# leftfield-geospatial/homonim

Measured on AMD Instinct MI355X. Metric: Mpixels*bands/s fit+apply (5x5 gain-offset, float32), higher is better.
Workload: dtype f32 in/out, f64 window sums; 1 GPU; synthetic float32 4-band 16384x16384 src/ref resident in HBM per GPU, Model.gain-offset, kernel 5x5, r2_inpaint_thresh 0.25, fused fit+apply (BASELINE.json configs[2]); bands=4, height=16384, width=16384, nodata_variant=0, parallelism=1 rank(s) x 1 GPU, one raster per rank, no collective

## Files before the change

### homonim_amd/csrc/hk_norm.hip

```cpp
#include "hk_kernels.h"

#include <type_traits>

namespace hk {

constexpr int NORM_THREADS = 256;
constexpr int L1_BITS = 11, L2_BITS = 11, L3_BITS = 10;
constexpr int L1_BINS = 1 << L1_BITS, L2_BINS = 1 << L2_BITS, L3_BINS = 1 << L3_BITS;
constexpr int SAMPLE_N = 4096;
#ifndef HK_NORM_ABLATE
#define HK_NORM_ABLATE 0
#endif
constexpr int PASS_WAVES = 2048;
constexpr int FB_BLOCKS = 512;
constexpr int MID_BLOCKS = 256;

struct Sel {
    unsigned prefix;
    unsigned long long rank;
};

struct NormWS {
    float lo[2], hi[2];
    double shift[2];
    unsigned sample_m;
    unsigned long long pn[PASS_WAVES], pbelow[2][PASS_WAVES];
    double p1[2][PASS_WAVES], p2[2][PASS_WAVES];
    unsigned mid_count[2];
    unsigned long long n;
    double mean[2], var[2], frac;
    unsigned long long k[2];
    int fallback, done;
    Sel sel[2][2];
    unsigned kbase[2];
    int ksh[2];
    float val[2][2];
    unsigned hist1[2][2][L1_BINS], hist2[2][2][L2_BINS], hist3[2][2][L3_BINS];
};

static_assert(sizeof(NormWS) == NORM_WS_BYTES, "the workspace's per-band piece (hk_layout.h)");

size_t norm_workspace_bytes(int n_bands, int height, int width) { return norm_layout(n_bands, height, width).total; }
static float* mid_buffers(void* workspace, const NormLayout& l) { return reinterpret_cast<float*>(static_cast<char*>(workspace) + l.mid); }

__device__ __forceinline__ unsigned f2key(float f) {
    const unsigned u = __float_as_uint(f);
    return (u & 0x80000000u) ? ~u : (u | 0x80000000u);
}
__device__ __forceinline__ float key2f(unsigned k) {
    const unsigned u = (k & 0x80000000u) ? (k & 0x7fffffffu) : ~k;
    return __uint_as_float(u);
}
__device__ __forceinline__ bool nvalid(float v, int mode, float nodata) {
    return mode == 0 ? true : (mode == 1 ? !(v != v) : !(v == nodata));
}

struct PlaneRef {
    const float* sp;
    const float* rp;
    long long stride;
    int height, width;
};
__device__ __forceinline__ PlaneRef plane_of(const NormArgs& a, int p) {
    PlaneRef r;
    if (a.planes != nullptr) {
        const __attribute__((address_space(1))) NormPlane* const e = (const __attribute__((address_space(1))) NormPlane*)a.planes + p;
        r.sp = e->src, r.rp = e->ref, r.stride = e->stride, r.height = e->height, r.width = e->width;
    } else {
        r.sp = a.src + (long long)p * a.band_stride, r.rp = a.ref + (long long)p * a.band_stride;
        r.stride = a.stride, r.height = a.height, r.width = a.width;
    }
    return r;
}

__device__ __forceinline__ float plane_at(const float* plane, long long i) {
    return *((__attribute__((address_space(1))) const float*)plane + i);
}

__device__ __forceinline__ double wave_sum(double v) {
#pragma unroll
    for (int d = WAVE / 2; d > 0; d >>= 1) v += __shfl_xor(v, d);
    return v;
}
__device__ __forceinline__ unsigned long long wave_sum(unsigned long long v) {
#pragma unroll
    for (int d = WAVE / 2; d > 0; d >>= 1) v += __shfl_xor(v, d);
    return v;
}

template <int NBINS, typename T = unsigned>
__device__ __forceinline__ bool select_bin(const T* __restrict__ h, unsigned long long rank, unsigned* bin_out,
                                           unsigned long long* rank_out) {
    const int lane = threadIdx.x & (WAVE - 1);
    constexpr int PER = NBINS / WAVE;
    unsigned v[PER];
    unsigned long long local = 0;
#pragma unroll
    for (int i = 0; i < PER; ++i) v[i] = h[lane * PER + i];
#pragma unroll
    for (int i = 0; i < PER; ++i) local += v[i];
    unsigned long long incl = local;
#pragma unroll
    for (int d = 1; d < WAVE; d <<= 1) {
        const unsigned long long u = __shfl_up(incl, d, WAVE);
        if (lane >= d) incl += u;
    }
    const unsigned long long hit = __ballot(incl > rank);
    const int owner = hit ? __ffsll(hit) - 1 : WAVE - 1;
    if (lane != owner) return false;
    unsigned long long cum = incl - local;
    int b = 0;
    bool found = false;
#pragma unroll
    for (int i = 0; i < PER - 1; ++i) {
        if (!found) {
            if (cum + v[i] > rank) found = true;
            else cum += v[i], b = i + 1;
        }
    }
    *bin_out = (unsigned)(lane * PER + b);
    *rank_out = rank - cum;
    return true;
}

constexpr int SAMPLE_THREADS = 256;
__global__ void __launch_bounds__(SAMPLE_THREADS) norm_sample_kernel(const NormArgs a, NormWS* __restrict__ ws_all) {
    static_assert(L1_BINS == L2_BINS && L3_BINS <= L1_BINS, "the sample select shares one histogram shape");
    static_assert(SAMPLE_N < 65536, "16-bit histogram counters");
    __shared__ float samp[SAMPLE_N];
    __shared__ unsigned hist[2][L1_BINS / 2];
    __shared__ unsigned cnt, spfx[2], srank[2];
    __shared__ int need[2];
    __shared__ double red[SAMPLE_THREADS / WAVE];
    const int band = blockIdx.x, t = threadIdx.x;
    NormWS& ws = ws_all[band];
    const PlaneRef pl = plane_of(a, band);
    const float* __restrict__ sp = pl.sp;
    const float* __restrict__ rp = pl.rp;
    const long long total = (long long)pl.height * pl.width;
    const long long step = total / SAMPLE_N > 0 ? total / SAMPLE_N : 1;
    for (int q = 0; q < 2; ++q) {
        if (t == 0) cnt = 0;
        for (int i = t; i < SAMPLE_N; i += SAMPLE_THREADS) samp[i] = __int_as_float(0x7f800000);
        __syncthreads();
        double sum = 0.0;
        for (int j = t; j < SAMPLE_N; j += SAMPLE_THREADS) {
            unsigned long long hsh = ((unsigned long long)j + 0x9e3779b97f4a7c15ull) * 0xbf58476d1ce4e5b9ull;
            hsh = (hsh ^ (hsh >> 29)) * 0x94d049bb133111ebull;
            hsh ^= hsh >> 32;
            const long long p = (long long)j * step + (long long)(hsh % (unsigned long long)step);
            if (p < total) {
                const int y = (int)(p / pl.width), x = (int)(p % pl.width);
                const float s = plane_at(sp, (long long)y * pl.stride + x), r = plane_at(rp, (long long)y * pl.stride + x);
                if (nvalid(s, a.src_nd_mode, a.src_nodata) && nvalid(r, a.ref_nd_mode, a.ref_nodata)) {
                    const float v = q ? r : s;
                    samp[atomicAdd(&cnt, 1u)] = v;
                    sum += (double)v;
                }
            }
        }
        __syncthreads();
        const unsigned m = cnt;
        {
            const double wsum = wave_sum(sum);
            if ((t & (WAVE - 1)) == 0) red[t / WAVE] = wsum;
        }
        if (t == 0) {
            const double c = 0.01 * (double)m, sd = sqrt(c > 0.0 ? c : 0.0);
            const long long ia = (long long)floor(c - 4.0 * sd) - 2, ib = (long long)ceil(c + 4.0 * sd) + 3;
            need[0] = !(m == 0 || ia <= 0), need[1] = !(m == 0 || ib >= (long long)m - 1);
            srank[0] = need[0] ? (unsigned)ia : 0u, srank[1] = need[1] ? (unsigned)ib : 0u;
            spfx[0] = spfx[1] = 0u;
        }
        __syncthreads();
        for (int level = 0; level < 3; ++level) {
            for (int i = t; i < L1_BINS; i += SAMPLE_THREADS) (&hist[0][0])[i] = 0;
            __syncthreads();
            for (int i = t; i < SAMPLE_N; i += SAMPLE_THREADS) {
                const unsigned key = f2key(samp[i]);
#pragma unroll
                for (int k = 0; k < 2; ++k) {
                    unsigned bin;
                    bool in;
                    if (level == 0) bin = key >> (32 - L1_BITS), in = true;
                    else if (level == 1) bin = (key >> L3_BITS) & (L2_BINS - 1), in = (key >> (32 - L1_BITS)) == spfx[k];
                    else bin = key & (L3_BINS - 1), in = (key >> L3_BITS) == spfx[k];
                    if (in) atomicAdd(&hist[k][bin >> 1], 1u << (16 * (bin & 1u)));
                }
            }
            __syncthreads();
            if (t < 2 * WAVE) {
                const int k = t / WAVE;
                const unsigned short* h16 = reinterpret_cast<const unsigned short*>(hist[k]);
                unsigned bin;
                unsigned long long rk;
                bool mine;
                if (level == 2) mine = select_bin<L3_BINS, unsigned short>(h16, srank[k], &bin, &rk);
                else mine = select_bin<L1_BINS, unsigned short>(h16, srank[k], &bin, &rk);
                if (mine) {
                    const int bits = level == 0 ? 0 : (level == 1 ? L2_BITS : L3_BITS);
                    spfx[k] = level == 0 ? bin : ((spfx[k] << bits) | bin);
                    srank[k] = (unsigned)rk;
                }
            }
            __syncthreads();
        }
        if (t == 0) {
            double s_all = 0.0;
            for (int i = 0; i < SAMPLE_THREADS / WAVE; ++i) s_all += red[i];
            const double mean = m ? s_all / (double)m : 0.0;
            ws.shift[q] = (mean == mean && fabs(mean) < 1e300) ? mean : 0.0;
            ws.sample_m = m;
            const float lo = key2f(spfx[0]), hi = key2f(spfx[1]);
            ws.lo[q] = need[0] ? (lo == 0.0f ? -0.0f : lo) : __int_as_float(0xff800000);
            ws.hi[q] = need[1] ? (hi == 0.0f ? 0.0f : hi) : __int_as_float(0x7f800000);
        }
        __syncthreads();
    }
}

constexpr size_t NORM_STREAM_LDS_PAD = 0;

__host__ __device__ static inline int pass_waves(int height, int width) {
    const long long chunks = (long long)height * (((width + PX - 1) / PX + WAVE - 1) / WAVE);
    long long w = chunks / 16;
    w = w < 64 ? 64 : (w > PASS_WAVES ? PASS_WAVES : w);
    return (int)w;
}

constexpr int QCAP = 16;

template <bool DENSE>
__global__ void __launch_bounds__(WAVE) norm_stream_kernel(const NormArgs a, NormWS* __restrict__ ws_all,
                                                            float* __restrict__ mid_all, size_t mid_cap) {
    __shared__ float stage[2][QCAP][WAVE];
    const int band = blockIdx.y, wave = blockIdx.x, lane = threadIdx.x;
    NormWS& ws = ws_all[band];
    const PlaneRef pl = plane_of(a, band);
    const int G = pass_waves(pl.height, pl.width);
    if (wave >= G) return;
    const float* __restrict__ sp = pl.sp;
    const float* __restrict__ rp = pl.rp;
    float* mid[2] = {mid_all + ((size_t)band * 2 + 0) * mid_cap, mid_all + ((size_t)band * 2 + 1) * mid_cap};
    const float lo[2] = {ws.lo[0], ws.lo[1]}, hi[2] = {ws.hi[0], ws.hi[1]};
    const double shift[2] = {ws.shift[0], ws.shift[1]};

    unsigned n = 0, le_hi[2] = {0, 0}, n_in[2] = {0, 0};
    double m1[2] = {0.0, 0.0}, m2[2] = {0.0, 0.0};
    unsigned cnt[2] = {0, 0};

    auto flush = [&](int q) {
        unsigned incl = cnt[q];
#pragma unroll
        for (int d = 1; d < WAVE; d <<= 1) {
            const unsigned v = __shfl_up(incl, d, WAVE);
            if (lane >= d) incl += v;
        }
        const unsigned total = __shfl(incl, WAVE - 1);
        unsigned base = 0;
        if (lane == 0) base = atomicAdd(&ws.mid_count[q], total);
        base = __shfl(base, 0);
        const size_t off = (size_t)base + (incl - cnt[q]);
        for (unsigned j = 0; j < cnt[q]; ++j)
            if (off + j < mid_cap) mid[q][off + j] = stage[q][j][lane];
        n_in[q] += cnt[q];
        cnt[q] = 0;
    };

    const int wq = (pl.width + PX - 1) / PX, cpr = (wq + WAVE - 1) / WAVE;
    const long long total = (long long)pl.height * cpr;
    const int dy = G / cpr, dc = G % cpr;
    int py = wave / cpr, pc = wave % cpr;
    long long pit = wave;
    auto fetch = [&](float4& s4, float4& r4, int& x) {
        const bool live = pit < total;
        const long long o = live ? (long long)py * pl.stride + (long long)pc * (WAVE * PX) : 0ll;
        const bool ok = live && pc * WAVE + lane < wq;
        const int lo4 = ok ? lane * PX : 0;
        typedef float f4v __attribute__((ext_vector_type(4)));
        typedef __attribute__((address_space(1))) const f4v gf4v;
        const f4v sv = __builtin_nontemporal_load((gf4v*)(sp + o + lo4));
        const f4v rv = __builtin_nontemporal_load((gf4v*)(rp + o + lo4));
        s4 = make_float4(sv.x, sv.y, sv.z, sv.w), r4 = make_float4(rv.x, rv.y, rv.z, rv.w);
        x = ok ? (pc * WAVE + lane) * PX : pl.width;
        pit += G, py += dy, pc += dc;
        if (pc >= cpr) pc -= cpr, ++py;
    };
    const float cmp_s = a.src_nd_mode == 2 ? a.src_nodata : __int_as_float(0x7fc00000);
    const float cmp_r = a.ref_nd_mode == 2 ? a.ref_nodata : __int_as_float(0x7fc00000);
    const bool nan_s = a.src_nd_mode == 1, nan_r = a.ref_nd_mode == 1;
    auto process = [&](const float4& s4, const float4& r4, int x, auto full) {
        constexpr bool FULL = decltype(full)::value;
        if (__any((cnt[0] > cnt[1] ? cnt[0] : cnt[1]) > (unsigned)(QCAP - PX))) {
            if (__any(cnt[0] > (unsigned)(QCAP - PX))) flush(0);
            if (__any(cnt[1] > (unsigned)(QCAP - PX))) flush(1);
        }
        const float s[PX] = {s4.x, s4.y, s4.z, s4.w}, r[PX] = {r4.x, r4.y, r4.z, r4.w};
        const int npx = pl.width - x;
#pragma unroll
        for (int i = 0; i < PX; ++i) {
            bool m = FULL || i < npx;
            if constexpr (!DENSE)
                m = m && !(s[i] == cmp_s) && !(r[i] == cmp_r) && (s[i] == s[i] || !nan_s) && (r[i] == r[i] || !nan_r);
            const float v[2] = {s[i], r[i]};
            if (m) {
                ++n;
#pragma unroll
                for (int q = 0; q < 2; ++q) {
                    if constexpr ((HK_NORM_ABLATE & 1) != 0) { m1[q] += (double)(v[q] == 1.2345f); continue; }
                    const double d = (double)v[q] - shift[q];
                    m1[q] += d;
                    m2[q] = __fma_rn(d, d, m2[q]);
                }
            }
#pragma unroll
            for (int q = 0; q < 2; ++q) {
                if constexpr ((HK_NORM_ABLATE & 2) != 0) { le_hi[q] += (m && v[q] <= hi[q]) ? 1u : 0u; continue; }
                const bool le = m && v[q] <= hi[q], in = le && !(v[q] < lo[q]);
                stage[q][cnt[q]][lane] = v[q];
                le_hi[q] += le ? 1u : 0u;
                cnt[q] += in ? 1u : 0u;
            }
        }
    };
    const bool quads = (pl.width % PX) == 0;
    auto process_any = [&](const float4& s4, const float4& r4, int x) {
        if (quads && __shfl(x, WAVE - 1) < pl.width) process(s4, r4, x, std::true_type{});
        else process(s4, r4, x, std::false_type{});
    };

    constexpr int NS = 3;
    float4 sQ[NS], rQ[NS];
    int xQ[NS];
#pragma unroll
    for (int k = 0; k < NS; ++k) fetch(sQ[k], rQ[k], xQ[k]);
    for (long long it = wave; it < total;) {
        bool more = true;
#pragma unroll
        for (int k = 0; k < NS; ++k) {
            if (more) {
                process_any(sQ[k], rQ[k], xQ[k]);
                fetch(sQ[k], rQ[k], xQ[k]);
                more = (it += G) < total;
            }
        }
    }
    flush(0);
    flush(1);
    const unsigned long long nw = wave_sum((unsigned long long)n);
    unsigned long long bw[2];
    for (int q = 0; q < 2; ++q) {
        m1[q] = wave_sum(m1[q]);
        m2[q] = wave_sum(m2[q]);
        bw[q] = wave_sum((unsigned long long)(le_hi[q] - n_in[q]));
    }
    if (lane == 0) {
        ws.pn[wave] = nw;
        for (int q = 0; q < 2; ++q) ws.p1[q][wave] = m1[q], ws.p2[q][wave] = m2[q], ws.pbelow[q][wave] = bw[q];
    }
}

constexpr int STATS_THREADS = 256;
__global__ void __launch_bounds__(STATS_THREADS) norm_stats_kernel(NormWS* __restrict__ ws_all, double* __restrict__ norm_out,
                                                                    size_t mid_cap) {
    static_assert(PASS_WAVES % STATS_THREADS == 0, "every thread sums the same number of partials");
    __shared__ unsigned long long sn[STATS_THREADS / WAVE], sb[2][STATS_THREADS / WAVE];
    __shared__ double s1[2][STATS_THREADS / WAVE], s2[2][STATS_THREADS / WAVE];
    NormWS& ws = ws_all[blockIdx.x];
    unsigned long long n = 0, below[2] = {0, 0};
    double m1[2] = {0.0, 0.0}, m2[2] = {0.0, 0.0};
#pragma unroll
    for (int j = 0; j < PASS_WAVES / STATS_THREADS; ++j) {
        const int i = threadIdx.x + j * STATS_THREADS;
        n += ws.pn[i];
#pragma unroll
        for (int q = 0; q < 2; ++q) m1[q] += ws.p1[q][i], m2[q] += ws.p2[q][i], below[q] += ws.pbelow[q][i];
    }
    n = wave_sum(n);
    for (int q = 0; q < 2; ++q) m1[q] = wave_sum(m1[q]), m2[q] = wave_sum(m2[q]), below[q] = wave_sum(below[q]);
    const int w = threadIdx.x / WAVE;
    if ((threadIdx.x & (WAVE - 1)) == 0) {
        sn[w] = n;
        for (int q = 0; q < 2; ++q) s1[q][w] = m1[q], s2[q][w] = m2[q], sb[q][w] = below[q];
    }
    __syncthreads();
    if (threadIdx.x != 0) return;
    n = 0;
    for (int q = 0; q < 2; ++q) m1[q] = m2[q] = 0.0, below[q] = 0;
    for (int i = 0; i < STATS_THREADS / WAVE; ++i) {
        n += sn[i];
        for (int q = 0; q < 2; ++q) m1[q] += s1[q][i], m2[q] += s2[q][i], below[q] += sb[q][i];
    }
    ws.n = n;
    if (n == 0) {
        norm_out[2 * blockIdx.x] = 0.0;
        norm_out[2 * blockIdx.x + 1] = 0.0;
        ws.done = 1;
        return;
    }
    for (int q = 0; q < 2; ++q) {
        const double d = m1[q] / (double)n;
        ws.mean[q] = ws.shift[q] + d;
        const double v = m2[q] / (double)n - d * d;
        ws.var[q] = v > 0.0 ? v : 0.0;
    }
    const double vi = 0.01 * (double)(n - 1);
    const unsigned long long k0 = (unsigned long long)floor(vi);
    ws.frac = vi - (double)k0;
    ws.k[0] = k0;
    ws.k[1] = k0 + 1 < n ? k0 + 1 : n - 1;
    int fb = 0;
    for (int q = 0; q < 2; ++q) {
        const unsigned long long nm = ws.mid_count[q];
        if (nm > mid_cap || ws.k[0] < below[q] || ws.k[1] >= below[q] + nm) fb = 1;
        ws.sel[q][0].rank = ws.k[0] - below[q];
        ws.sel[q][1].rank = ws.k[1] - below[q];
        ws.sel[q][0].prefix = ws.sel[q][1].prefix = 0;
        const unsigned kb = f2key(ws.lo[q]), range = f2key(ws.hi[q]) - kb;
        ws.kbase[q] = kb;
        ws.ksh[q] = range ? __clz((int)range) : 0;
    }
    if (fb)
        for (int q = 0; q < 2; ++q) {
            ws.sel[q][0].rank = ws.k[0], ws.sel[q][1].rank = ws.k[1];
            ws.kbase[q] = 0, ws.ksh[q] = 0;
        }
    ws.fallback = fb;
}

__device__ __forceinline__ void hist_add(unsigned* hist, int level, unsigned key, const unsigned (&pfx)[2]) {
    if (level == 0) {
        atomicAdd(&hist[key >> (32 - L1_BITS)], 1u);
        return;
    }
#pragma unroll
    for (int k = 0; k < 2; ++k) {
        if (level == 1) {
            if ((key >> (32 - L1_BITS)) == pfx[k]) atomicAdd(&hist[k * L2_BINS + ((key >> L3_BITS) & (L2_BINS - 1))], 1u);
        } else {
            if ((key >> L3_BITS) == pfx[k]) atomicAdd(&hist[k * L3_BINS + (key & (L3_BINS - 1))], 1u);
        }
    }
}

template <int LEVEL>
__global__ void __launch_bounds__(NORM_THREADS) norm_mid_hist_kernel(const NormArgs a, NormWS* __restrict__ ws_all,
                                                                       const float* __restrict__ mid_all, size_t mid_cap) {
    constexpr int NB = LEVEL == 0 ? L1_BINS : (LEVEL == 1 ? L2_BINS : L3_BINS);
    __shared__ unsigned hist[2 * NB];
    const int band = blockIdx.y >> 1, q = blockIdx.y & 1;
    NormWS& ws = ws_all[band];
    if (ws.done) return;
    for (int i = threadIdx.x; i < 2 * NB; i += NORM_THREADS) hist[i] = 0;
    __syncthreads();
    if (ws.fallback) {
        const PlaneRef pl = plane_of(a, band);
        const unsigned pfx[2] = {ws.sel[q][0].prefix, ws.sel[q][1].prefix};
        const unsigned kb = ws.kbase[q];
        const int ksh = ws.ksh[q];
        for (int y = blockIdx.x; y < pl.height; y += gridDim.x) {
            const long long row = (long long)y * pl.stride;
            for (int x = threadIdx.x; x < pl.width; x += NORM_THREADS) {
                const float s = plane_at(pl.sp, row + x), r = plane_at(pl.rp, row + x);
                if (nvalid(s, a.src_nd_mode, a.src_nodata) && nvalid(r, a.ref_nd_mode, a.ref_nodata))
                    hist_add(hist, LEVEL, (f2key(q ? r : s) - kb) << ksh, pfx);
            }
        }
        __syncthreads();
        unsigned* gh = LEVEL == 0 ? &ws.hist1[q][0][0] : (LEVEL == 1 ? &ws.hist2[q][0][0] : &ws.hist3[q][0][0]);
        for (int i = threadIdx.x; i < 2 * NB; i += NORM_THREADS)
            if (hist[i]) atomicAdd(gh + i, hist[i]);
        return;
    }
    const float* __restrict__ buf = mid_all + ((size_t)band * 2 + q) * mid_cap;
    const unsigned cnt = ws.mid_count[q];
    const unsigned pfx[2] = {ws.sel[q][0].prefix, ws.sel[q][1].prefix};
    const unsigned kb = ws.kbase[q];
    const int ksh = ws.ksh[q];
    auto rel = [&](float v) { return (f2key(v) - kb) << ksh; };
    const float4* __restrict__ buf4 = reinterpret_cast<const float4*>(buf);
    const unsigned cnt4 = cnt >> 2;
    for (unsigned i = blockIdx.x * NORM_THREADS + threadIdx.x; i < cnt4; i += gridDim.x * NORM_THREADS) {
        const float4 v = buf4[i];
        hist_add(hist, LEVEL, rel(v.x), pfx), hist_add(hist, LEVEL, rel(v.y), pfx);
        hist_add(hist, LEVEL, rel(v.z), pfx), hist_add(hist, LEVEL, rel(v.w), pfx);
    }
    if (blockIdx.x == 0 && threadIdx.x < (cnt & 3u)) hist_add(hist, LEVEL, rel(buf[(cnt & ~3u) + threadIdx.x]), pfx);
    __syncthreads();
    unsigned* gh = LEVEL == 0 ? &ws.hist1[q][0][0] : (LEVEL == 1 ? &ws.hist2[q][0][0] : &ws.hist3[q][0][0]);
    for (int i = threadIdx.x; i < 2 * NB; i += NORM_THREADS)
        if (hist[i]) atomicAdd(gh + i, hist[i]);
}

template <int LEVEL>
__global__ void __launch_bounds__(NORM_THREADS) norm_full_hist_kernel(const NormArgs a, NormWS* __restrict__ ws_all) {
    constexpr int NB = LEVEL == 0 ? L1_BINS : (LEVEL == 1 ? L2_BINS : L3_BINS);
    __shared__ unsigned hist[2 * NB];
    const int band = blockIdx.y, q = blockIdx.z;
    NormWS& ws = ws_all[band];
    if (ws.done || !ws.fallback) return;
    for (int i = threadIdx.x; i < 2 * NB; i += NORM_THREADS) hist[i] = 0;
    __syncthreads();
    const PlaneRef pl = plane_of(a, band);
    const float* __restrict__ sp = pl.sp;
    const float* __restrict__ rp = pl.rp;
    const unsigned pfx[2] = {ws.sel[q][0].prefix, ws.sel[q][1].prefix};
    const unsigned kb = ws.kbase[q];
    const int ksh = ws.ksh[q];
    for (int y = blockIdx.x; y < pl.height; y += gridDim.x) {
        const long long row = (long long)y * pl.stride;
        for (int x = threadIdx.x; x < pl.width; x += NORM_THREADS) {
            const float s = plane_at(sp, row + x), r = plane_at(rp, row + x);
            if (nvalid(s, a.src_nd_mode, a.src_nodata) && nvalid(r, a.ref_nd_mode, a.ref_nodata))
                hist_add(hist, LEVEL, (f2key(q ? r : s) - kb) << ksh, pfx);
        }
    }
    __syncthreads();
    unsigned* gh = LEVEL == 0 ? &ws.hist1[q][0][0] : (LEVEL == 1 ? &ws.hist2[q][0][0] : &ws.hist3[q][0][0]);
    for (int i = threadIdx.x; i < 2 * NB; i += NORM_THREADS)
        if (hist[i]) atomicAdd(gh + i, hist[i]);
}

template <int LEVEL>
__global__ void __launch_bounds__(NORM_THREADS) norm_select_kernel(NormWS* __restrict__ ws_all, double* __restrict__ norm_out) {
    static_assert(NORM_THREADS == 4 * WAVE, "one wave per (raster, rank)");
    NormWS& ws = ws_all[blockIdx.x];
    if (ws.done) return;
    {
        const int q = threadIdx.x >> 7, k = (threadIdx.x >> 6) & 1;
        const unsigned* h = LEVEL == 0 ? ws.hist1[q][0] : (LEVEL == 1 ? ws.hist2[q][k] : ws.hist3[q][k]);
        constexpr int NB = LEVEL == 0 ? L1_BINS : (LEVEL == 1 ? L2_BINS : L3_BINS);
        unsigned bin;
        unsigned long long rk;
        if (select_bin<NB>(h, ws.sel[q][k].rank, &bin, &rk)) {
            const int bits = LEVEL == 0 ? 0 : (LEVEL == 1 ? L2_BITS : L3_BITS);
            ws.sel[q][k].prefix = (LEVEL == 0) ? bin : ((ws.sel[q][k].prefix << bits) | bin);
            ws.sel[q][k].rank = rk;
            if (LEVEL == 2) ws.val[q][k] = key2f((ws.sel[q][k].prefix >> ws.ksh[q]) + ws.kbase[q]);
        }
    }
    __syncthreads();
    if (LEVEL == 2 && threadIdx.x == 0) {
        const double n0 = sqrt(ws.var[1]) / sqrt(ws.var[0]);
        double pct[2];
        for (int q = 0; q < 2; ++q) {
            const double lo = (double)ws.val[q][0], hi = (double)ws.val[q][1], t = ws.frac;
            const double d = hi - lo;
            pct[q] = t >= 0.5 ? hi - d * (1.0 - t) : lo + d * t;
        }
        norm_out[2 * blockIdx.x] = n0;
        norm_out[2 * blockIdx.x + 1] = pct[1] - pct[0] * n0;
    }
}

constexpr int SPLIT_XCHG = 4 * L1_BINS;

size_t norm_split_exchange_doubles(int n_bands) { return (size_t)n_bands * SPLIT_XCHG; }

__global__ void split_put_shift_kernel(NormWS* __restrict__ ws_all, double* __restrict__ xchg) {
    NormWS& ws = ws_all[blockIdx.x];
    double* x = xchg + (size_t)blockIdx.x * SPLIT_XCHG;
    for (int i = threadIdx.x; i < SPLIT_XCHG; i += blockDim.x) x[i] = i < 2 ? ws.shift[i] : (i == 2 && ws.sample_m ? 1.0 : 0.0);
}
__global__ void split_get_shift_kernel(NormWS* __restrict__ ws_all, const double* __restrict__ xchg) {
    if (threadIdx.x != 0) return;
    NormWS& ws = ws_all[blockIdx.x];
    const double* x = xchg + (size_t)blockIdx.x * SPLIT_XCHG;
    for (int q = 0; q < 2; ++q) {
        ws.shift[q] = x[2] > 0.0 ? x[q] / x[2] : 0.0;
        ws.lo[q] = ws.hi[q] = __int_as_float(0xff800000);
    }
}
__global__ void split_put_moments_kernel(NormWS* __restrict__ ws_all, double* __restrict__ xchg) {
    NormWS& ws = ws_all[blockIdx.x];
    unsigned long long n = 0;
    double m1[2] = {0.0, 0.0}, m2[2] = {0.0, 0.0};
    for (int i = threadIdx.x; i < PASS_WAVES; i += WAVE) {
        n += ws.pn[i];
        for (int q = 0; q < 2; ++q) m1[q] += ws.p1[q][i], m2[q] += ws.p2[q][i];
    }
    n = wave_sum(n);
    for (int q = 0; q < 2; ++q) m1[q] = wave_sum(m1[q]), m2[q] = wave_sum(m2[q]);
    if (threadIdx.x != 0) return;
    double* x = xchg + (size_t)blockIdx.x * SPLIT_XCHG;
    x[0] = (double)n, x[1] = m1[0], x[2] = m2[0], x[3] = m1[1], x[4] = m2[1];
}
__global__ void split_get_moments_kernel(NormWS* __restrict__ ws_all, const double* __restrict__ xchg,
                                         double* __restrict__ norm_out) {
    if (threadIdx.x != 0) return;
    NormWS& ws = ws_all[blockIdx.x];
    const double* x = xchg + (size_t)blockIdx.x * SPLIT_XCHG;
    const unsigned long long n = (unsigned long long)x[0];
    ws.n = n;
    ws.mid_count[0] = ws.mid_count[1] = 0;
    if (n == 0) {
        norm_out[2 * blockIdx.x] = 0.0, norm_out[2 * blockIdx.x + 1] = 0.0;
        ws.done = 1;
        return;
    }
    if (n >= (1ull << 32)) {
        const double qn = __longlong_as_double(0x7ff8000000000000ll);
        norm_out[2 * blockIdx.x] = qn, norm_out[2 * blockIdx.x + 1] = qn;
        ws.done = 1;
        return;
    }
    for (int q = 0; q < 2; ++q) {
        const double d = x[1 + 2 * q] / (double)n;
        ws.mean[q] = ws.shift[q] + d;
        const double v = x[2 + 2 * q] / (double)n - d * d;
        ws.var[q] = v > 0.0 ? v : 0.0;
    }
    const double vi = 0.01 * (double)(n - 1);
    const unsigned long long k0 = (unsigned long long)floor(vi);
    ws.frac = vi - (double)k0;
    ws.k[0] = k0, ws.k[1] = k0 + 1 < n ? k0 + 1 : n - 1;
    for (int q = 0; q < 2; ++q)
        for (int k = 0; k < 2; ++k) ws.sel[q][k].rank = ws.k[k], ws.sel[q][k].prefix = 0;
    ws.fallback = 1;
}
template <int LEVEL>
__global__ void split_hist_kernel(NormWS* __restrict__ ws_all, double* __restrict__ xchg, int put) {
    constexpr int NB = LEVEL == 0 ? L1_BINS : (LEVEL == 1 ? L2_BINS : L3_BINS);
    NormWS& ws = ws_all[blockIdx.x];
    unsigned* h = LEVEL == 0 ? &ws.hist1[0][0][0] : (LEVEL == 1 ? &ws.hist2[0][0][0] : &ws.hist3[0][0][0]);
    double* x = xchg + (size_t)blockIdx.x * SPLIT_XCHG;
    for (int i = threadIdx.x; i < SPLIT_XCHG; i += blockDim.x) {
        if (put) x[i] = i < 4 * NB ? (double)h[i] : 0.0;
        else if (i < 4 * NB) h[i] = (unsigned)x[i];
    }
}

hipError_t launch_block_norm_split(const NormArgs& a, void* workspace, double* xchg, int phase,
                                   double* norm_out, hipStream_t stream) {
    NormWS* ws = reinterpret_cast<NormWS*>(workspace);
    const dim3 bands(a.n_bands), block(NORM_THREADS), gfull(FB_BLOCKS, a.n_bands, 2);
    const bool rows = a.height > 0;
    switch (phase) {
    case 0: {
        hipError_t e = hipMemsetAsync(ws, 0, sizeof(NormWS) * (size_t)a.n_bands, stream);
        if (e != hipSuccess) return e;
        if (rows) HK_LAUNCH(norm_sample_kernel, bands, dim3(SAMPLE_THREADS), 0, stream, a, ws);
        HK_LAUNCH(split_put_shift_kernel, bands, block, 0, stream, ws, xchg);
        break;
    }
    case 1: {
        HK_LAUNCH(split_get_shift_kernel, bands, dim3(WAVE), 0, stream, ws, xchg);
        if (rows) {
            const dim3 gstream(pass_waves(a.height, a.width), a.n_bands);
            const NormLayout lay = norm_layout(a.n_bands, a.height, a.width);
            float* mid = mid_buffers(workspace, lay);
            const size_t cap_al = lay.cap_al;
            if (a.src_nd_mode == 0 && a.ref_nd_mode == 0)
                HK_LAUNCH(norm_stream_kernel<true>, gstream, dim3(WAVE), NORM_STREAM_LDS_PAD, stream, a, ws, mid, cap_al);
            else
                HK_LAUNCH(norm_stream_kernel<false>, gstream, dim3(WAVE), NORM_STREAM_LDS_PAD, stream, a, ws, mid, cap_al);
        }
        HK_LAUNCH(split_put_moments_kernel, bands, dim3(WAVE), 0, stream, ws, xchg);
        break;
    }
    case 2:
        HK_LAUNCH(split_get_moments_kernel, bands, dim3(WAVE), 0, stream, ws, xchg, norm_out);
        if (rows) HK_LAUNCH(norm_full_hist_kernel<0>, gfull, block, 0, stream, a, ws);
        HK_LAUNCH(split_hist_kernel<0>, bands, block, 0, stream, ws, xchg, 1);
        break;
    case 3:
        HK_LAUNCH(split_hist_kernel<0>, bands, block, 0, stream, ws, xchg, 0);
        HK_LAUNCH(norm_select_kernel<0>, bands, block, 0, stream, ws, norm_out);
        if (rows) HK_LAUNCH(norm_full_hist_kernel<1>, gfull, block, 0, stream, a, ws);
        HK_LAUNCH(split_hist_kernel<1>, bands, block, 0, stream, ws, xchg, 1);
        break;
    case 4:
        HK_LAUNCH(split_hist_kernel<1>, bands, block, 0, stream, ws, xchg, 0);
        HK_LAUNCH(norm_select_kernel<1>, bands, block, 0, stream, ws, norm_out);
        if (rows) HK_LAUNCH(norm_full_hist_kernel<2>, gfull, block, 0, stream, a, ws);
        HK_LAUNCH(split_hist_kernel<2>, bands, block, 0, stream, ws, xchg, 1);
        break;
    case 5:
        HK_LAUNCH(split_hist_kernel<2>, bands, block, 0, stream, ws, xchg, 0);
        HK_LAUNCH(norm_select_kernel<2>, bands, block, 0, stream, ws, norm_out);
        break;
    default:
        return hipErrorInvalidValue;
    }
    return hipGetLastError();
}

int norm_pass_waves(int height, int width) { return pass_waves(height, width); }

hipError_t launch_block_norm(const NormArgs& a, void* workspace, double* norm_out, hipStream_t stream) {
    NormWS* ws = reinterpret_cast<NormWS*>(workspace);
    const NormLayout lay = norm_layout(a.n_bands, a.height, a.width);
    float* mid = mid_buffers(workspace, lay);
    const size_t cap_al = lay.cap_al;
    hipError_t e = hipMemsetAsync(ws, 0, sizeof(NormWS) * (size_t)a.n_bands, stream);
    if (e != hipSuccess) return e;
    const dim3 bands(a.n_bands), block(NORM_THREADS);
    HK_LAUNCH(norm_sample_kernel, bands, dim3(SAMPLE_THREADS), 0, stream, a, ws);
    const dim3 gstream(a.grid_waves > 0 ? a.grid_waves : pass_waves(a.height, a.width), a.n_bands);
    if (a.src_nd_mode == 0 && a.ref_nd_mode == 0)
        HK_LAUNCH(norm_stream_kernel<true>, gstream, dim3(WAVE), NORM_STREAM_LDS_PAD, stream, a, ws, mid, cap_al);
    else
        HK_LAUNCH(norm_stream_kernel<false>, gstream, dim3(WAVE), NORM_STREAM_LDS_PAD, stream, a, ws, mid, cap_al);
    HK_LAUNCH(norm_stats_kernel, bands, dim3(STATS_THREADS), 0, stream, ws, norm_out, cap_al);
    const size_t mid_wgs = cap_al / 4 / (NORM_THREADS * 8);
    const dim3 gmid((unsigned)(mid_wgs < 32 ? 32 : (mid_wgs > MID_BLOCKS ? MID_BLOCKS : mid_wgs)), a.n_bands * 2);
    HK_LAUNCH(norm_mid_hist_kernel<0>, gmid, block, 0, stream, a, ws, mid, cap_al);
    HK_LAUNCH(norm_select_kernel<0>, bands, block, 0, stream, ws, norm_out);
    HK_LAUNCH(norm_mid_hist_kernel<1>, gmid, block, 0, stream, a, ws, mid, cap_al);
    HK_LAUNCH(norm_select_kernel<1>, bands, block, 0, stream, ws, norm_out);
    HK_LAUNCH(norm_mid_hist_kernel<2>, gmid, block, 0, stream, a, ws, mid, cap_al);
    HK_LAUNCH(norm_select_kernel<2>, bands, block, 0, stream, ws, norm_out);
    return hipGetLastError();
}

}
```

Baseline: 368,700 Mpixels*bands/s.

## Restructure norm sample kernel into a single register-resident pass and drop the memset

The sample kernel now gathers each thread's 16 sample positions once, loads src and ref together into registers, and builds both rasters' radix-select histograms in one pass, so it no longer runs two serial passes through a shared-memory sample array with atomic compaction. Padding is added as a single weighted count instead of filling with +inf. Sample position math gets a 32-bit fast path that avoids 64-bit modulo when the step is small. The workspace zeroing moves into the kernel, replacing a separate hipMemsetAsync. This is a small per-band prelude kernel, so the effect on whole fit+apply throughput is likely minor.

```diff
diff --git a/homonim_amd/csrc/hk_norm.hip b/homonim_amd/csrc/hk_norm.hip
--- a/homonim_amd/csrc/hk_norm.hip
+++ b/homonim_amd/csrc/hk_norm.hip
@@ -1,5 +1,8 @@
 #include "hk_kernels.h"
 
+#include "hk_norm_pos.h"
+
+#include <stddef.h>
 #include <type_traits>
 
 namespace hk {
@@ -124,98 +127,125 @@
 }
 
 constexpr int SAMPLE_THREADS = 256;
-__global__ void __launch_bounds__(SAMPLE_THREADS) norm_sample_kernel(const NormArgs a, NormWS* __restrict__ ws_all) {
+constexpr int SAMPLE_PER = SAMPLE_N / SAMPLE_THREADS;
+__global__ void __launch_bounds__(SAMPLE_THREADS, 4) norm_sample_kernel(const NormArgs a, NormWS* __restrict__ ws_all) {
     static_assert(L1_BINS == L2_BINS && L3_BINS <= L1_BINS, "the sample select shares one histogram shape");
     static_assert(SAMPLE_N < 65536, "16-bit histogram counters");
-    __shared__ float samp[SAMPLE_N];
-    __shared__ unsigned hist[2][L1_BINS / 2];
-    __shared__ unsigned cnt, spfx[2], srank[2];
+    static_assert(SAMPLE_N == NORM_SAMPLE_N && SAMPLE_PER <= 32, "hk_norm_pos.h; one validity bit per position");
+    static_assert(SAMPLE_THREADS == 4 * WAVE, "one wave per (raster, rank)");
+    __shared__ unsigned hist[2][2][L1_BINS / 2];
+    __shared__ unsigned spfx[2][2], srank[2][2], scnt[SAMPLE_THREADS / WAVE];
     __shared__ int need[2];
-    __shared__ double red[SAMPLE_THREADS / WAVE];
+    __shared__ double red[2][SAMPLE_THREADS / WAVE];
     const int band = blockIdx.x, t = threadIdx.x;
     NormWS& ws = ws_all[band];
+    {
+        static_assert(offsetof(NormWS, pn) % 8 == 0 && sizeof(NormWS) % 8 == 0, "cleared by 8-byte stores");
+        constexpr int NZ = (int)((sizeof(NormWS) - offsetof(NormWS, pn)) / 8);
+        unsigned long long* z = reinterpret_cast<unsigned long long*>(reinterpret_cast<char*>(&ws) + offsetof(NormWS, pn));
+        for (int i = t; i < NZ; i += SAMPLE_THREADS) z[i] = 0ull;
+    }
     const PlaneRef pl = plane_of(a, band);
-    const float* __restrict__ sp = pl.sp;
-    const float* __restrict__ rp = pl.rp;
-    const long long total = (long long)pl.height * pl.width;
-    const long long step = total / SAMPLE_N > 0 ? total / SAMPLE_N : 1;
-    for (int q = 0; q < 2; ++q) {
-        if (t == 0) cnt = 0;
-        for (int i = t; i < SAMPLE_N; i += SAMPLE_THREADS) samp[i] = __int_as_float(0x7f800000);
+    const SampleGeom g = sample_geom(pl.height, pl.width);
+    long long off[SAMPLE_PER];
+    unsigned in = 0;
+    if (g.narrow) {
+#pragma unroll
+        for (int i = 0; i < SAMPLE_PER; ++i) {
+            const SamplePos pos = sample_pos_narrow(g, t + i * SAMPLE_THREADS);
+            const bool inside = pos.p < g.total;
+            off[i] = inside ? (long long)pos.y * pl.stride + pos.x : 0ll;
+            in |= inside ? 1u << i : 0u;
+        }
+    } else {
+#pragma unroll
+        for (int k = 0; k < SAMPLE_PER; ++k) off[k] = 0ll;
+#pragma unroll 1
+        for (int i = 0; i < SAMPLE_PER; ++i) {
+            const SamplePos pos = sample_pos_wide(g, t + i * SAMPLE_THREADS);
+            const bool inside = pos.p < g.total;
+            const long long o = inside ? (long long)pos.y * pl.stride + pos.x : 0ll;
+#pragma unroll
+            for (int k = 0; k < SAMPLE_PER; ++k) off[k] = k == i ? o : off[k];
+            in |= inside ? 1u << i : 0u;
+        }
+    }
+    float v[2][SAMPLE_PER];
+#pragma unroll
+    for (int i = 0; i < SAMPLE_PER; ++i) v[0][i] = plane_at(pl.sp, off[i]), v[1][i] = plane_at(pl.rp, off[i]);
+    unsigned ok = 0;
+    double sum[2] = {0.0, 0.0};
+#pragma unroll
+    for (int i = 0; i < SAMPLE_PER; ++i)
+        if ((in & (1u << i)) && nvalid(v[0][i], a.src_nd_mode, a.src_nodata) && nvalid(v[1][i], a.ref_nd_mode, a.ref_nodata)) {
+            ok |= 1u << i;
+            sum[0] += (double)v[0][i], sum[1] += (double)v[1][i];
+        }
+    {
+        const unsigned long long wcnt = wave_sum((unsigned long long)__popc(ok));
+        const double w0 = wave_sum(sum[0]), w1 = wave_sum(sum[1]);
+        if ((t & (WAVE - 1)) == 0) scnt[t / WAVE] = (unsigned)wcnt, red[0][t / WAVE] = w0, red[1][t / WAVE] = w1;
+    }
+    __syncthreads();
+    unsigned m = 0;
+    for (int i = 0; i < SAMPLE_THREADS / WAVE; ++i) m += scnt[i];
+    if (t == 0) {
+        const double c = 0.01 * (double)m, sd = sqrt(c > 0.0 ? c : 0.0);
+        const long long ia = (long long)floor(c - 4.0 * sd) - 2, ib = (long long)ceil(c + 4.0 * sd) + 3;
+        need[0] = !(m == 0 || ia <= 0), need[1] = !(m == 0 || ib >= (long long)m - 1);
+        for (int q = 0; q < 2; ++q) {
+            srank[q][0] = need[0] ? (unsigned)ia : 0u, srank[q][1] = need[1] ? (unsigned)ib : 0u;
+            spfx[q][0] = spfx[q][1] = 0u;
+        }
+    }
+    const unsigned pad = SAMPLE_N - m, pad_key = f2key(__int_as_float(0x7f800000));
+    for (int level = 0; level < 3; ++level) {
+        for (int i = t; i < 2 * L1_BINS; i += SAMPLE_THREADS) (&hist[0][0][0])[i] = 0;
         __syncthreads();
-        double sum = 0.0;
-        for (int j = t; j < SAMPLE_N; j += SAMPLE_THREADS) {
-            unsigned long long hsh = ((unsigned long long)j + 0x9e3779b97f4a7c15ull) * 0xbf58476d1ce4e5b9ull;
-            hsh = (hsh ^ (hsh >> 29)) * 0x94d049bb133111ebull;
-            hsh ^= hsh >> 32;
-            const long long p = (long long)j * step + (long long)(hsh % (unsigned long long)step);
-            if (p < total) {
-                const int y = (int)(p / pl.width), x = (int)(p % pl.width);
-                const float s = plane_at(sp, (long long)y * pl.stride + x), r = plane_at(rp, (long long)y * pl.stride + x);
-                if (nvalid(s, a.src_nd_mode, a.src_nodata) && nvalid(r, a.ref_nd_mode, a.ref_nodata)) {
-                    const float v = q ? r : s;
-                    samp[atomicAdd(&cnt, 1u)] = v;
-                    sum += (double)v;
-                }
+        const unsigned pfx[4] = {spfx[0][0], spfx[0][1], spfx[1][0], spfx[1][1]};
+        const int sh = level == 0 ? 32 - L1_BITS : (level == 1 ? L3_BITS : 0), psh = level == 1 ? 32 - L1_BITS : L3_BITS;
+        const unsigned mask = level == 2 ? L3_BINS - 1 : L1_BINS - 1;
+        auto add = [&](auto raster, unsigned key, unsigned count) {
+            constexpr int Q = decltype(raster)::value;
+#pragma unroll
+            for (int k = 0; k < 2; ++k) {
+                const unsigned bin = (key >> sh) & mask;
+                if (level == 0 || (key >> psh) == pfx[Q * 2 + k]) atomicAdd(&hist[Q][k][bin >> 1], count << (16 * (bin & 1u)));
             }
-        }
+        };
+        const std::integral_constant<int, 0> src_raster;
+        const std::integral_constant<int, 1> ref_raster;
+#pragma unroll
+        for (int i = 0; i < SAMPLE_PER; ++i)
+            if (ok & (1u << i)) add(src_raster, f2key(v[0][i]), 1u), add(ref_raster, f2key(v[1][i]), 1u);
+        if (t == 0 && pad) add(src_raster, pad_key, pad), add(ref_raster, pad_key, pad);
         __syncthreads();
-        const unsigned m = cnt;
         {
-            const double wsum = wave_sum(sum);
-            if ((t & (WAVE - 1)) == 0) red[t / WAVE] = wsum;
-        }
-        if (t == 0) {
-            const double c = 0.01 * (double)m, sd = sqrt(c > 0.0 ? c : 0.0);
-            const long long ia = (long long)floor(c - 4.0 * sd) - 2, ib = (long long)ceil(c + 4.0 * sd) + 3;
-            need[0] = !(m == 0 || ia <= 0), need[1] = !(m == 0 || ib >= (long long)m - 1);
-            srank[0] = need[0] ? (unsigned)ia : 0u, srank[1] = need[1] ? (unsigned)ib : 0u;
-            spfx[0] = spfx[1] = 0u;
+            const int q = t / (2 * WAVE), k = (t / WAVE) & 1;
+            const unsigned short* h16 = reinterpret_cast<const unsigned short*>(hist[q][k]);
+            unsigned bin;
+            unsigned long long rk;
+            bool mine;
+            if (level == 2) mine = select_bin<L3_BINS, unsigned short>(h16, srank[q][k], &bin, &rk);
+            else mine = select_bin<L1_BINS, unsigned short>(h16, srank[q][k], &bin, &rk);
+            if (mine) {
+                const int bits = level == 0 ? 0 : (level == 1 ? L2_BITS : L3_BITS);
+                spfx[q][k] = level == 0 ? bin : ((spfx[q][k] << bits) | bin);
+                srank[q][k] = (unsigned)rk;
+            }
         }
         __syncthreads();
-        for (int level = 0; level < 3; ++level) {
-            for (int i = t; i < L1_BINS; i += SAMPLE_THREADS) (&hist[0][0])[i] = 0;
-            __syncthreads();
-            for (int i = t; i < SAMPLE_N; i += SAMPLE_THREADS) {
-                const unsigned key = f2key(samp[i]);
-#pragma unroll
-                for (int k = 0; k < 2; ++k) {
-                    unsigned bin;
-                    bool in;
-                    if (level == 0) bin = key >> (32 - L1_BITS), in = true;
-                    else if (level == 1) bin = (key >> L3_BITS) & (L2_BINS - 1), in = (key >> (32 - L1_BITS)) == spfx[k];
-                    else bin = key & (L3_BINS - 1), in = (key >> L3_BITS) == spfx[k];
-                    if (in) atomicAdd(&hist[k][bin >> 1], 1u << (16 * (bin & 1u)));
-                }
-            }
-            __syncthreads();
-            if (t < 2 * WAVE) {
-                const int k = t / WAVE;
-                const unsigned short* h16 = reinterpret_cast<const unsigned short*>(hist[k]);
-                unsigned bin;
-                unsigned long long rk;
-                bool mine;
-                if (level == 2) mine = select_bin<L3_BINS, unsigned short>(h16, srank[k], &bin, &rk);
-                else mine = select_bin<L1_BINS, unsigned short>(h16, srank[k], &bin, &rk);
-                if (mine) {
-                    const int bits = level == 0 ? 0 : (level == 1 ? L2_BITS : L3_BITS);
-                    spfx[k] = level == 0 ? bin : ((spfx[k] << bits) | bin);
-                    srank[k] = (unsigned)rk;
-                }
-            }
-            __syncthreads();
-        }
-        if (t == 0) {
-            double s_all = 0.0;
-            for (int i = 0; i < SAMPLE_THREADS / WAVE; ++i) s_all += red[i];
-            const double mean = m ? s_all / (double)m : 0.0;
-            ws.shift[q] = (mean == mean && fabs(mean) < 1e300) ? mean : 0.0;
-            ws.sample_m = m;
-            const float lo = key2f(spfx[0]), hi = key2f(spfx[1]);
-            ws.lo[q] = need[0] ? (lo == 0.0f ? -0.0f : lo) : __int_as_float(0xff800000);
-            ws.hi[q] = need[1] ? (hi == 0.0f ? 0.0f : hi) : __int_as_float(0x7f800000);
-        }
-        __syncthreads();
+    }
+    if (t < 2) {
+        const int q = t;
+        double s_all = 0.0;
+        for (int i = 0; i < SAMPLE_THREADS / WAVE; ++i) s_all += red[q][i];
+        const double mean = m ? s_all / (double)m : 0.0;
+        ws.shift[q] = (mean == mean && fabs(mean) < 1e300) ? mean : 0.0;
+        if (q == 0) ws.sample_m = m;
+        const float lo = key2f(spfx[q][0]), hi = key2f(spfx[q][1]);
+        ws.lo[q] = need[0] ? (lo == 0.0f ? -0.0f : lo) : __int_as_float(0xff800000);
+        ws.hi[q] = need[1] ? (hi == 0.0f ? 0.0f : hi) : __int_as_float(0x7f800000);
     }
 }
 
@@ -692,8 +722,6 @@
     const NormLayout lay = norm_layout(a.n_bands, a.height, a.width);
     float* mid = mid_buffers(workspace, lay);
     const size_t cap_al = lay.cap_al;
-    hipError_t e = hipMemsetAsync(ws, 0, sizeof(NormWS) * (size_t)a.n_bands, stream);
-    if (e != hipSuccess) return e;
     const dim3 bands(a.n_bands), block(NORM_THREADS);
     HK_LAUNCH(norm_sample_kernel, bands, dim3(SAMPLE_THREADS), 0, stream, a, ws);
     const dim3 gstream(a.grid_waves > 0 ? a.grid_waves : pass_waves(a.height, a.width), a.n_bands);
diff --git a/homonim_amd/csrc/hk_norm_pos.h b/homonim_amd/csrc/hk_norm_pos.h
--- /dev/null
+++ b/homonim_amd/csrc/hk_norm_pos.h
@@ -0,0 +1,63 @@
+#pragma once
+
+#if defined(__HIPCC__) || defined(__CUDACC__)
+#define HK_POS_FN __host__ __device__ inline
+#else
+#define HK_POS_FN inline
+#endif
+
+namespace hk {
+
+constexpr int NORM_SAMPLE_N = 4096;
+
+struct SamplePos {
+    long long p;
+    int y, x;
+};
+
+HK_POS_FN unsigned long long sample_hash(int j) {
+    unsigned long long hsh = ((unsigned long long)j + 0x9e3779b97f4a7c15ull) * 0xbf58476d1ce4e5b9ull;
+    hsh = (hsh ^ (hsh >> 29)) * 0x94d049bb133111ebull;
+    hsh ^= hsh >> 32;
+    return hsh;
+}
+
+struct SampleGeom {
+    long long total, step;
+    int width;
+    bool narrow;
+    unsigned step32, pow32_mod;
+};
+
+HK_POS_FN SampleGeom sample_geom(int height, int width) {
+    SampleGeom g;
+    g.total = (long long)height * width;
+    g.step = g.total / NORM_SAMPLE_N > 0 ? g.total / NORM_SAMPLE_N : 1;
+    g.width = width;
+    g.narrow = g.step <= 65536;
+    g.step32 = g.narrow ? (unsigned)g.step : 1u;
+    g.pow32_mod = (unsigned)((1ull << 32) % (unsigned long long)g.step32);
+    return g;
+}
+
+HK_POS_FN SamplePos sample_pos_wide(const SampleGeom& g, int j) {
+    SamplePos r;
+    r.p = (long long)j * g.step + (long long)(sample_hash(j) % (unsigned long long)g.step);
+    r.y = (int)(r.p / g.width), r.x = (int)(r.p % g.width);
+    return r;
+}
+
+HK_POS_FN SamplePos sample_pos_narrow(const SampleGeom& g, int j) {
+    const unsigned long long hsh = sample_hash(j);
+    const unsigned hi = (unsigned)(hsh >> 32), lo = (unsigned)hsh;
+    const unsigned rem = ((hi % g.step32) * g.pow32_mod + lo % g.step32) % g.step32;
+    const unsigned p = (unsigned)j * g.step32 + rem;
+    SamplePos r;
+    r.p = (long long)p;
+    r.y = (int)(p / (unsigned)g.width), r.x = (int)(p % (unsigned)g.width);
+    return r;
+}
+
+HK_POS_FN SamplePos sample_pos(const SampleGeom& g, int j) { return g.narrow ? sample_pos_narrow(g, j) : sample_pos_wide(g, j); }
+
+}
```

Result: slower. 364,300 Mpixels*bands/s (-1.2%).
